# nkkk98/MyGPURaytracer

Hardware: AMD Instinct MI355X
Metric: Mrays/s (higher is better)
Workload: dtype f32; 1 GPU; cornellObj.txt 1920x1080 depth 8, AA on, material sort on, 1 spp/step (BASELINE configs[3] / C4); arith=0, clock_warmup_steps=1152, rccl_ranks=1, parallelism=1 GPU

## Files before the change

### include/mi355x_pathtracer.h

```cpp
#ifndef MI355X_PATHTRACER_H
#define MI355X_PATHTRACER_H

#include <stddef.h>
#include <stdint.h>

#ifdef __cplusplus
extern "C" {
#endif

#define PTX_ABI_VERSION 5
int ptx_abi_version(void);
size_t ptx_sizeof_options(void);
size_t ptx_sizeof_stats(void);

#define PTX_OK 0
#define PTX_ERR_INVALID 1
#define PTX_ERR_IO 2
#define PTX_ERR_HIP 3
#define PTX_ERR_NODEVICE 4
#define PTX_ERR_UNSUPPORTED 5

enum { PTX_SPHERE = 0, PTX_CUBE = 1, PTX_TRIANGLE = 2, PTX_OBJ = 3 };

typedef struct ptx_material {
// ... 212 lines not shown
int  ptx_moments_add(ptx_moments *m, ptx_tracer *t, int64_t samples_total);
int  ptx_moments_add_host(ptx_moments *m, const float *host_rgb_sum, int64_t samples_total);
int  ptx_moments_read(ptx_moments *m, float *mean3, float *cov6, int32_t *batches1, int64_t *samples_out);
int  ptx_moments_summarize(ptx_moments *m, const ptx_moments_params *p, ptx_moments_summary *out);
int  ptx_denoise_measured(ptx_tracer *t, ptx_moments *m, const ptx_denoise_params *dp, const ptx_variance_params *vp, int min_batches,
                          int spp);

int ptx_kat_geom_test(ptx_tracer *t, int geom, int n, const float *rays6, float *out10);
int ptx_kat_obj_tri_test(ptx_tracer *t, int geom, int n, const float *rays6, float *out8);
int ptx_kat_jittered_hemisphere(ptx_tracer *t, int n, const float *normals3, const int32_t *seeds3, int max_iter, float *out3);
int ptx_kat_compute_intersections(ptx_tracer *t, int n, const void *paths44, void *isects32);
int ptx_kat_tile_intersect(ptx_tracer *t, int n, const void *paths44, void *isects32, int split);
int ptx_kat_shade(ptx_tracer *t, int iter, int n, const int32_t *idx, const void *isects32, void *paths44);
int ptx_kat_generate(ptx_tracer *t, int iter, void *paths44);
int ptx_kat_libm(ptx_tracer *t, int n, const float *x, float *sin_out, float *cos_out,
                 const double *pw_in, double *pow5_out, const float *powf_xy, float *powf_out);
int ptx_kat_fast_exact(ptx_tracer *t, int64_t mismatches[3]);
int ptx_debug_tile_geoms(const ptx_camera *camera, int ngeoms, const float *boxes6, int depth_of_field, int tile_rows, int tile_rank,
                         int tile_world, uint32_t *masks_out, int max_tiles);
int ptx_debug_record_masks(int nmaterials, const ptx_material *materials, int ngeoms, const int32_t *geom_type, const int32_t *geom_material,
                           int sort_by_material, uint64_t masks[2]);
int ptx_debug_cull_boxes(int n, const float *boxes6, float *centre_half8);
int ptx_debug_light_bits(int nmaterials, const ptx_material *materials, int ngeoms, const int32_t *geom_material, uint32_t *bits_out);
#define PTX_WALK_LOOP 0
#define PTX_WALK_SKIP 1
#define PTX_WALK_ORDERED 2
#define PTX_WALK_WIDE 3
#define PTX_WALK_WIDE_REFILL 4
int ptx_debug_mesh_plan(ptx_tracer *t, int geom, int32_t out8[8]);
int ptx_debug_bounce_occupancy(ptx_tracer *t, int lds_bytes);
int ptx_debug_aux_nonzero(ptx_tracer *t, int64_t out3[3]);
int ptx_debug_set_capture(ptx_tracer *t, int bounce);
int ptx_debug_bvh_check(const float *faces15, int nfaces, const float *rays6, int nrays, int32_t *face_loop, float *t_loop,
                        int32_t *face_bvh, float *t_bvh, int64_t *stats4);
int ptx_debug_bvh_visits(int64_t out8[8]);
int ptx_debug_read_stamps(ptx_tracer *t, unsigned long long out48[48]);
int ptx_debug_read_stream(ptx_tracer *t, int *n_out, int32_t *pixel_index, int32_t *stream_idx,
                          int32_t *material, float *fields14, int cap);

#ifdef __cplusplus
}
#endif
#endif
```

### mygpuraytracer_amd/api.py

```python
import ctypes as C
import os
import sys
import subprocess

import numpy as np

PKG_DIR = os.path.dirname(os.path.abspath(__file__))
LIB_PATH = os.path.join(PKG_DIR, "libmi355x_pathtracer.so")
if os.environ.get("PTX_AB_LIBRARY"):
    if os.environ.get("PTX_DEV") != "1":
        raise ImportError("PTX_AB_LIBRARY is set (%s) without PTX_DEV=1: variant builds are loaded for A/B timing only; unset it or "
                          "set PTX_DEV=1" % os.environ["PTX_AB_LIBRARY"])
    LIB_PATH = os.path.abspath(os.environ["PTX_AB_LIBRARY"])

PTX_OK = 0
ABI_VERSION = 5
vp = C.c_void_p


class PathTracerError(RuntimeError):
    pass


class Material(C.Structure):
# ... 230 lines not shown
    n = L.ptx_debug_tile_geoms(C.byref(camera), len(b), _ptr(b), int(bool(depth_of_field)), rows, rank, world, _ptr(out), cap)
    if n < 0:
        raise PathTracerError("ptx_debug_tile_geoms: bad argument")
    return out[:n]


def debug_cull_boxes(boxes6):
    L = load_library()
    b = np.ascontiguousarray(boxes6, np.float32).reshape(-1, 6)
    out = np.zeros((len(b), 8), np.float32)
    if L.ptx_debug_cull_boxes(len(b), _ptr(b), _ptr(out)) < 0:
        raise PathTracerError("ptx_debug_cull_boxes: bad argument")
    return out


def debug_light_bits(materials, geom_material):
    L = load_library()
    m = np.ascontiguousarray(materials, np.float32).reshape(-1, 11)
    gm = np.ascontiguousarray(geom_material, np.int32).reshape(-1)
    out = np.zeros(1, np.uint32)
    if L.ptx_debug_light_bits(len(m), _ptr(m), len(gm), _ptr(gm), _ptr(out)) < 0:
        raise PathTracerError("ptx_debug_light_bits: bad argument")
    return int(out[0])


WALK_NAMES = ("loop", "skip", "ordered", "wide", "wide_refill")


def build_library(force=False):
    if force or not os.path.exists(LIB_PATH):
        subprocess.check_call(["make", "-s", "-C", os.path.join(PKG_DIR, "csrc")])
    return LIB_PATH


_lib = None


class Orbit(C.Structure):
    _fields_ = [("phi", C.c_float), ("theta", C.c_float), ("zoom", C.c_float), ("og_look_at", C.c_float * 3)]


def _share_hip_runtime_with_torch():
    import importlib.util
    if "torch" in sys.modules:
        return
    try:
# ... 117 lines not shown
    L.ptx_moments_summarize.restype, L.ptx_moments_summarize.argtypes = i, [vp, C.POINTER(MomentsParams), C.POINTER(MomentsSummary)]
    L.ptx_denoise_measured.restype = i
    L.ptx_denoise_measured.argtypes = [vp, vp, C.POINTER(DenoiseParams), C.POINTER(VarianceParams), i, i]
    L.ptx_get_stats.restype, L.ptx_get_stats.argtypes = i, [vp, C.POINTER(Stats)]
    L.ptx_get_stats_sized.restype, L.ptx_get_stats_sized.argtypes = i, [vp, vp, C.c_size_t]
    L.ptx_owned_pixels.restype, L.ptx_owned_pixels.argtypes = i, [vp]
    L.ptx_stream.restype, L.ptx_stream.argtypes = vp, [vp]
    L.ptx_set_kernel_timing.restype, L.ptx_set_kernel_timing.argtypes = i, [vp, i]
    L.ptx_get_kernel_times.restype, L.ptx_get_kernel_times.argtypes = i, [vp, vp, vp]
    L.ptx_kat_geom_test.restype, L.ptx_kat_geom_test.argtypes = i, [vp, i, i, vp, vp]
    L.ptx_kat_compute_intersections.restype, L.ptx_kat_compute_intersections.argtypes = i, [vp, i, vp, vp]
    L.ptx_kat_obj_tri_test.restype, L.ptx_kat_obj_tri_test.argtypes = i, [vp, i, i, vp, vp]
    L.ptx_kat_jittered_hemisphere.restype, L.ptx_kat_jittered_hemisphere.argtypes = i, [vp, i, vp, vp, i, vp]
    L.ptx_kat_tile_intersect.restype, L.ptx_kat_tile_intersect.argtypes = i, [vp, i, vp, vp, i]
    L.ptx_kat_shade.restype, L.ptx_kat_shade.argtypes = i, [vp, i, i, vp, vp, vp]
    L.ptx_kat_generate.restype, L.ptx_kat_generate.argtypes = i, [vp, i, vp]
    L.ptx_kat_libm.restype, L.ptx_kat_libm.argtypes = i, [vp, i, vp, vp, vp, vp, vp, vp, vp]
    if hasattr(L, "ptx_debug_tile_geoms"):
        L.ptx_debug_tile_geoms.restype, L.ptx_debug_tile_geoms.argtypes = i, [vp, i, vp, i, i, i, i, vp, i]
    if hasattr(L, "ptx_debug_cull_boxes"):
        L.ptx_debug_cull_boxes.restype, L.ptx_debug_cull_boxes.argtypes = i, [i, vp, vp]
    if hasattr(L, "ptx_debug_light_bits"):
        L.ptx_debug_light_bits.restype, L.ptx_debug_light_bits.argtypes = i, [i, vp, i, vp, vp]
    if hasattr(L, "ptx_debug_mesh_plan"):
        L.ptx_debug_mesh_plan.restype, L.ptx_debug_mesh_plan.argtypes = i, [vp, i, vp]
    if hasattr(L, "ptx_kat_fast_exact"):
        L.ptx_kat_fast_exact.restype, L.ptx_kat_fast_exact.argtypes = i, [vp, vp]
    L.ptx_debug_set_capture.restype, L.ptx_debug_set_capture.argtypes = i, [vp, i]
    L.ptx_debug_read_stream.restype, L.ptx_debug_read_stream.argtypes = i, [vp, C.POINTER(i), vp, vp, vp, vp, i]
    L.ptx_multi_create.restype, L.ptx_multi_create.argtypes = i, [vp, C.POINTER(Options), C.POINTER(C.c_int), i, i, C.POINTER(vp)]
    L.ptx_multi_destroy.argtypes = [vp]
    L.ptx_multi_device_count.restype, L.ptx_multi_device_count.argtypes = i, [vp]
    L.ptx_multi_tracer.restype, L.ptx_multi_tracer.argtypes = vp, [vp, i]
    L.ptx_multi_set_camera.restype, L.ptx_multi_set_camera.argtypes = i, [vp, C.POINTER(Camera), i]
    for n in ("ptx_multi_reset_image", "ptx_multi_synchronize", "ptx_multi_assemble"):
        getattr(L, n).restype, getattr(L, n).argtypes = i, [vp]
    L.ptx_multi_iterate.restype, L.ptx_multi_iterate.argtypes = i, [vp, i]
    L.ptx_multi_set_render_ahead.restype, L.ptx_multi_set_render_ahead.argtypes = i, [vp, i]
    L.ptx_multi_render.restype, L.ptx_multi_render.argtypes = i, [vp, i, i]
    L.ptx_multi_device_image.restype, L.ptx_multi_device_image.argtypes = vp, [vp]
    L.ptx_multi_read_image.restype, L.ptx_multi_read_image.argtypes = i, [vp, vp]
    L.ptx_multi_read_albedo.restype, L.ptx_multi_read_albedo.argtypes = i, [vp, vp]
    L.ptx_multi_get_stats.restype, L.ptx_multi_get_stats.argtypes = i, [vp, C.POINTER(Stats)]
    L.ptx_pin_host_buffer.restype, L.ptx_pin_host_buffer.argtypes = i, [vp, C.c_size_t]
    L.ptx_unpin_host_buffer.restype, L.ptx_unpin_host_buffer.argtypes = i, [vp]
    L.sc_cpu_scan.argtypes = [i, vp, vp]
# ... 666 lines not shown
```

### mygpuraytracer_amd/csrc/pt_device.h

```cpp
#pragma once
#include <hip/hip_runtime.h>
#include <stdint.h>

#define PT_DEV __device__ __forceinline__
#define PT_HD __host__ __device__ __forceinline__

#ifndef PT_ARITH
#define PT_ARITH 0
#endif

namespace ptd {

struct vec3 { float x, y, z; };

PT_HD vec3 V3(float x, float y, float z) { vec3 r; r.x = x; r.y = y; r.z = z; return r; }
PT_HD vec3 add(vec3 a, vec3 b) { return V3(a.x + b.x, a.y + b.y, a.z + b.z); }
PT_HD vec3 sub(vec3 a, vec3 b) { return V3(a.x - b.x, a.y - b.y, a.z - b.z); }
PT_HD vec3 mul(vec3 a, vec3 b) { return V3(a.x * b.x, a.y * b.y, a.z * b.z); }
PT_HD vec3 scale(vec3 a, float s) { return V3(a.x * s, a.y * s, a.z * s); }
PT_HD vec3 neg(vec3 a) { return V3(-a.x, -a.y, -a.z); }
PT_HD float dot(vec3 a, vec3 b) { return a.x * b.x + a.y * b.y + a.z * b.z; }
PT_HD vec3 cross(vec3 x, vec3 y) { return V3(x.y * y.z - y.y * x.z, x.z * y.x - y.z * x.x, x.x * y.y - y.x * x.y); }
#ifndef PT_FAST_EXACT
#define PT_FAST_EXACT 1
// ... 249 lines not shown
    const float *__restrict__ tri9;
    const uint8_t *__restrict__ texels;
    int32_t ngeoms, nmats;
    int32_t tri_lds;
    int32_t ntri;
    int32_t ntri_lds;
    const float *__restrict__ gtab;
    const float *__restrict__ aabb;
    uint32_t cube_bits, sphere_bits, mesh_bits;
    uint32_t light_bits;
    const BvhQuad *__restrict__ bvh_nodes;
    const float *__restrict__ bvh_tris;
    const int32_t *__restrict__ bvh_root;
    const int32_t *__restrict__ bvh_depth;
    int32_t bvh_stack;
    const BvhWide4 *__restrict__ bvh_wide;
    const int32_t *__restrict__ bvh_wroot;
    const int32_t *__restrict__ bvh_wneed;
    const float *__restrict__ fnorm;
    const float *__restrict__ cnorm;
    uint32_t bump_bits;
    int32_t mesh_chunks;
    int32_t cull;
    const float *__restrict__ ldsblob;
};

__host__ __device__ constexpr int sceneTableWords(int ntri_lds, int nmats, int ngeoms) { return (ntri_lds * 27 + nmats * 11 + ngeoms * 58 + 3) & ~3; }
PT_DEV int sceneLdsWords(const DScene &sc) { return sceneTableWords(sc.ntri_lds, sc.nmats, sc.ngeoms); }
constexpr int GTAB_WORDS = 40;

extern __shared__ __attribute__((aligned(16))) int32_t pt_lds[];

__device__ __forceinline__ void stageSceneToLds(const DScene &sc, int tid, int nthreads) {
    float *l = reinterpret_cast<float *>(pt_lds);
    if (sc.ldsblob) {
        const int n = sc.ntri_lds * 27 + sc.nmats * 11 + sc.ngeoms * 58;
        for (int k = tid; k < n; k += 4 * nthreads) {
            const int k1 = k + nthreads, k2 = k1 + nthreads, k3 = k2 + nthreads;
            const float a0 = sc.ldsblob[k], a1 = k1 < n ? sc.ldsblob[k1] : 0.f, a2 = k2 < n ? sc.ldsblob[k2] : 0.f, a3 = k3 < n ? sc.ldsblob[k3] : 0.f;
            l[k] = a0;
            if (k1 < n) l[k1] = a1;
            if (k2 < n) l[k2] = a2;
            if (k3 < n) l[k3] = a3;
        }
        return;
    }
    const int n9 = sc.ntri_lds * 9, n15 = sc.ntri_lds * 15, nm = sc.nmats * 11;
// ... 557 lines not shown
    }
    if (hit_geom_index != -1) {
        const DGeom &geom = sc.geoms[hit_geom_index];
        h.t = t_min;
        h.geom = hit_geom_index;
        h.mat = geom.materialid;
        h.u = best.u; h.v = best.v;
        if (geom.type == G_CUBE) h.n = boxNormal(geom, best);
        else if (geom.type == G_SPHERE) h.n = sphereNormal(geom, best);
        else { vec3 geoN; h.n = meshNormal(sc, geom, best, geoN); }
    }
}


PT_HD vec3 mulRows(const float *r, vec3 v, float w) {
    vec3 o;
    o.x = (r[0] * v.x + r[1] * v.y) + (r[2] * v.z + r[3] * w);
    o.y = (r[4] * v.x + r[5] * v.y) + (r[6] * v.z + r[7] * w);
    o.z = (r[8] * v.x + r[9] * v.y) + (r[10] * v.z + r[11] * w);
    return o;
}

constexpr float CULL_FAR_ORIGIN = 1024.0f;
template <bool SUBSET = false>
PT_DEV uint32_t cullMask(const DScene &sc, Ray ray, uint32_t subset = 0xffffffffu) {
    typedef const __attribute__((address_space(4))) float cfloat;
    cfloat *ab = (cfloat *)sc.aabb;
    const float tiny = 1e-20f;
    const float ddx = __builtin_fabsf(ray.d.x) < tiny ? __builtin_copysignf(tiny, ray.d.x) : ray.d.x;
    const float ddy = __builtin_fabsf(ray.d.y) < tiny ? __builtin_copysignf(tiny, ray.d.y) : ray.d.y;
    const float ddz = __builtin_fabsf(ray.d.z) < tiny ? __builtin_copysignf(tiny, ray.d.z) : ray.d.z;
    const float ix = __builtin_amdgcn_rcpf(ddx), iy = __builtin_amdgcn_rcpf(ddy), iz = __builtin_amdgcn_rcpf(ddz);
    const float ox = -(ray.o.x * ix), oy = -(ray.o.y * iy), oz = -(ray.o.z * iz);
    const float ax = __builtin_fabsf(ix), ay = __builtin_fabsf(iy), az = __builtin_fabsf(iz);
    uint32_t mask = 0;
    const int n = sc.ngeoms;
    auto far_origin = [&]() {
        return __builtin_fmaxf(__builtin_fmaxf(__builtin_fabsf(ray.o.x), __builtin_fabsf(ray.o.y)), __builtin_fabsf(ray.o.z)) > CULL_FAR_ORIGIN;
    };
    auto slab = [&](const float *bx) {
        const float mx = __builtin_fmaf(bx[0], ix, ox), my = __builtin_fmaf(bx[1], iy, oy), mz = __builtin_fmaf(bx[2], iz, oz);
        const float x0 = __builtin_fmaf(bx[4], -ax, mx), x1 = __builtin_fmaf(bx[4], ax, mx);
        const float y0 = __builtin_fmaf(bx[5], -ay, my), y1 = __builtin_fmaf(bx[5], ay, my);
        const float z0 = __builtin_fmaf(bx[6], -az, mz), z1 = __builtin_fmaf(bx[6], az, mz);
        const float tn = __builtin_fmaxf(__builtin_fmaxf(x0, y0), z0);
        const float tf = __builtin_fminf(__builtin_fminf(x1, y1), z1);
        return !((tf < tn) || (tf < 0.0f));
    };
    if (SUBSET) {
        uint32_t todo = __builtin_amdgcn_readfirstlane(n >= 32 ? subset : subset & ((1u << n) - 1u));
        while (todo) {
            const int i = __builtin_ctz(todo);
            todo &= todo - 1;
            const int j = todo ? __builtin_ctz(todo) : i;
            todo &= todo - 1;
            float bx[2][8];
#pragma unroll
            for (int k = 0; k < 8; k++) { bx[0][k] = ab[i * 8 + k]; bx[1][k] = ab[j * 8 + k]; }
            mask |= slab(bx[0]) ? (1u << i) : 0u;
            mask |= slab(bx[1]) ? (1u << j) : 0u;
        }
        if (sc.cull > 1 && far_origin()) mask = n >= 32 ? subset : subset & ((1u << n) - 1u);
        return mask;
    }
    int i = n - 1;
    if (n & 1) {
        float bx[8];
#pragma unroll
        for (int k = 0; k < 8; k++) bx[k] = ab[i * 8 + k];
        mask = slab(bx) ? 1u : 0u;
        i--;
    }
    for (; i > 0; i -= 2) {
        float bx[2][8];
#pragma unroll
        for (int k = 0; k < 8; k++) { bx[0][k] = ab[i * 8 + k]; bx[1][k] = ab[(i - 1) * 8 + k]; }
#pragma unroll
        for (int h = 0; h < 2; h++) {
            const unsigned long long verdict = __builtin_amdgcn_ballot_w64(slab(bx[h]));
            asm("v_addc_co_u32_e64 %0, vcc, %0, %0, %1" : "+v"(mask) : "s"(verdict) : "vcc");
        }
    }
    if (sc.cull > 1 && far_origin()) mask = n >= 32 ? 0xffffffffu : (1u << n) - 1u;
    return mask;
}

constexpr unsigned long long KEY_NONE = ~0ull;
PT_DEV unsigned long long packKey(float t, int g, uint32_t aux) {
    return ((unsigned long long)(uint32_t)__float_as_int(t) << 32) | ((unsigned long long)(uint32_t)g << 24) | (aux & 0xffffffu);
}

PT_DEV unsigned long long primKey(const float *gtab, int g, Ray ray) {
    const float *G = gtab + g * GTAB_WORDS;
    float inv[12];
#pragma unroll
    for (int k = 0; k < 12; k++) inv[k] = G[k];
    const int type = __float_as_int(G[36]);
    Ray q;
    q.o = mulRows(inv, ray.o, 1.0f);
    q.d = normalize(mulRows(inv, ray.d, 0.0f));
    vec3 objP = V3(0.f, 0.f, 0.f);
    uint32_t aux = 0;
    bool hit = false;
    if (type == G_CUBE) {
        float tmin = -1e38f, tmax = 1e38f;
// ... 426 lines not shown
```

### mygpuraytracer_amd/csrc/pt_engine.hip

```cpp
#include <hip/hip_runtime.h>
#include <stdint.h>
#include <stdio.h>
#include <string.h>
#include <string>
#include <vector>
#include <algorithm>
#include <cmath>

#include "../../include/mi355x_pathtracer.h"
#include "pt_kernels.h"
#include "pt_scene.h"
#include "pt_denoise.h"

namespace {

thread_local std::string g_last_error;
int set_error(int code, const std::string &msg) { g_last_error = msg; return code; }

#define HIPCHECK(expr)                                                                                   \
    do {                                                                                                 \
        hipError_t e_ = (expr);                                                                          \
        if (e_ != hipSuccess)                                                                            \
            return set_error(PTX_ERR_HIP, std::string(#expr) + ": " + hipGetErrorString(e_));            \
    } while (0)
// ... 205 lines not shown
    hipEvent_t ev_start = nullptr, ev_stop = nullptr;
    bool timing_valid = false;
    ptx_options opt{};
    DCamera cam{};
    int traceDepth = 0;
    TileMap tm{};
    int nbins = 1, nmats = 0, ngeoms = 0, maxTiles = 0, grid = 0, grid_seg = 0, cap = 0, cus = 0;
    bool grid_forced = false;
    int dbg_mesh_wg_per_cu = 0;
    int dbg_extra_lds = 0;
    int dbg_total_wg_per_cu = 0, dbg_nsets = 0;
    DevBuf<DGeom> d_geoms; DevBuf<DMaterial> d_mats; DevBuf<float> d_faces; DevBuf<uint8_t> d_texels;
    float *d_image = nullptr; DevBuf<float> d_image_own;
    DevBuf<float> d_fbuf[3];
    DevBuf<int32_t> d_ibuf[3];
    PathSoA soa[3];
    DevBuf<int32_t> d_counts;
    DevBuf<int32_t> d_chunk;
    DevBuf<int32_t> d_cache_chunk;
    DevBuf<int32_t> d_cache_super;
    int cache_gx = 0;
    DevBuf<int32_t> d_totals;
    int32_t *d_super = nullptr;
    DevBuf<float> d_tri9, d_gtab, d_aabb;
    std::vector<float> h_aabb;
    std::vector<int32_t> h_geom_type, h_roots, h_depths, h_wroots, h_wneeds;
    DevBuf<uint32_t> d_tile_geoms; bool tile_geoms_valid = false;
    DevBuf<BvhQuad> d_bvh_nodes; DevBuf<float> d_bvh_tris; DevBuf<int32_t> d_bvh_root, d_bvh_depth;
    DevBuf<BvhWide4> d_bvh_wide; DevBuf<int32_t> d_bvh_wroot, d_bvh_wneed;
    DevBuf<float> d_fnorm, d_cnorm;
    DevBuf<float> d_ldsblob;
    bool no_fast = false;
    bool no_last = false;
    bool force_fast = false;
    DevBuf<unsigned long long> d_keys; DevBuf<uint32_t> d_items; DevBuf<int32_t> d_item_count;
    DevBuf<int32_t> d_tile_done;
    size_t seg_items = 0;
    int nsuper = 1;
    size_t totals_bytes = 0, seg_totals = 0, field_stride = 0, seg_part = 0;
    int kmax = 1;
    long long split_min_paths = 1LL << 20;
    int lanes = 1;
    hipStream_t lane_stream[MAX_LANES] = {};
    hipEvent_t ev_fork = nullptr, ev_join[MAX_LANES] = {}, ev_chain[MAX_LANES] = {};
    struct Ahead { int first = 0, count = 0, next = 0, unfolded = 0; bool use_cache = false, valid = false, timed = false;
                   unsigned long long dir_bins = ~0ull, ntab_bins = 0ull; };
    Ahead ahead[MAX_LANES];
// ... 15 lines not shown
    DevBuf<float> d_var;
    bool var_done = false;
    DevBuf<unsigned long long> d_stamps;
    DevBuf<float> d_part;
    DevBuf<int32_t> d_cache_totals;
    DevBuf<int32_t> d_emit_count, d_emit_pix; DevBuf<float> d_emit_rgb;
    DevBuf<int64_t> d_stats;
    uint32_t fence_slots = 0;
    int maxBounces = 0;
    bool cache_valid = false;
    int64_t iterations = 0;
    double loop_ms_total = 0.0;
    bool ktiming = false;
    std::vector<hipEvent_t> kev;
    std::vector<int> kev_kind;
    size_t kev_used = 0;
    int capture_bounce = -1;
    DevBuf<int32_t> d_cap;
    DevBuf<float> d_cap_f;
    bool cap_filled = false;
    DScene scene() const {
        DScene s; s.geoms = d_geoms; s.mats = d_mats; s.faces = d_faces; s.tri9 = d_tri9; s.texels = d_texels; s.ngeoms = ngeoms; s.nmats = nmats;
        s.gtab = d_gtab; s.aabb = d_aabb; s.cull = 0; s.cube_bits = cube_bits; s.sphere_bits = sphere_bits; s.mesh_bits = mesh_bits; s.light_bits = light_bits;
        s.bvh_nodes = d_bvh_nodes; s.bvh_tris = d_bvh_tris; s.bvh_root = d_bvh_root; s.bvh_depth = d_bvh_depth; s.bvh_wide = d_bvh_wide; s.bvh_wroot = d_bvh_wroot; s.bvh_wneed = d_bvh_wneed; s.bvh_stack = 0; s.ntri_lds = 0; s.mesh_chunks = mesh_chunks;
        s.fnorm = d_fnorm; s.cnorm = d_cnorm; s.bump_bits = bump_bits;
        s.tri_lds = 0; s.ntri = ntri;
        s.ldsblob = nullptr;
        return s;
    }
    bool cache_active() const { return opt.cache_first_bounce && !opt.antialiasing && !opt.depth_of_field; }
    const KernelSet *ks = static_cast<const KernelSet *>(ptx_arith_kernels_0());
    const LastKernelSet *ksl = static_cast<const LastKernelSet *>(ptx_arith_last_0());
};

namespace {

void carve(PathSoA &s, float *f, int32_t *i, size_t stride) {
    s.q = f; s.i = i; s.stride = (uint32_t)stride;
}

PathSoA soa_shift(PathSoA s, size_t off) {
    s.q += 4 * off; s.i += off;
    return s;
}

void fastdiv_magic(uint32_t d, uint32_t &mul, uint32_t &sh) {
// ... 443 lines not shown
    HC(hipGetDeviceProperties(&prop, dev));
    camera_to_device(*camera, t->cam);
    const int W = t->cam.resx, H = t->cam.resy;
    t->tm.W = W; t->tm.H = H; t->tm.tile_world = opt.tile_world; t->tm.tile_rank = opt.tile_rank;
    t->tm.tile_rows = opt.tile_world > 1 ? opt.tile_rows : H;
    fastdiv_magic((uint32_t)W, t->tm.w_mul, t->tm.w_sh);
    fastdiv_magic((uint32_t)t->tm.tile_rows, t->tm.rows_mul, t->tm.rows_sh);
    t->tm.owned = owned_pixels(W, H, t->tm.tile_rows, opt.tile_rank, opt.tile_world);
    t->maxTiles = (std::max(t->tm.owned, 1) + TILE - 1) / TILE;
    t->cap = t->maxTiles * TILE;
    t->nbins = opt.sort_by_material ? (nmaterials > 0 ? nmaterials : 1) : 1;
    {
        int per_cu = 16;
        if (const char *e = getenv("PTX_DEBUG_WG_PER_CU")) { per_cu = std::max(1, atoi(e)); t->grid_forced = true; }
        t->cus = prop.multiProcessorCount;
        t->grid = std::max(1, std::min(t->maxTiles, prop.multiProcessorCount * per_cu));
    }
    t->grid_seg = std::max(1, std::min(t->grid, t->maxTiles));
    t->nsuper = (t->grid_seg + 63) / 64;
    HostScene hs;
    SceneSwitches sw;
    sw.no_wide_bvh = getenv("PTX_DEBUG_NO_WIDE_BVH") != nullptr; sw.no_chunks = getenv("PTX_DEBUG_NO_CHUNKS") != nullptr;
    sw.no_dir_skip = getenv("PTX_DEBUG_NO_DIR_SKIP") != nullptr; sw.no_normal_codes = getenv("PTX_DEBUG_NO_NORMAL_CODES") != nullptr;
    sw.force_split = getenv("PTX_DEBUG_FORCE_SPLIT") != nullptr;
    if (const int rc = pt_prepare_scene(ngeoms, geoms, nmaterials, materials, opt, t->tm.owned, t->nbins, prop.sharedMemPerBlock, sw, hs)) return fail(rc);
    static_cast<SceneFacts &>(*t) = hs;
    {
        size_t mem_free = 0, mem_total = 0;
        if (opt.batch <= 0 && hipMemGetInfo(&mem_free, &mem_total) != hipSuccess) { mem_free = mem_total = 0; (void)hipGetLastError(); }
        const char *e = getenv("PTX_DEBUG_MEM_BUDGET_MB");
        const LaunchPlan plan = plan_launch_sets(t->tm.owned, t->nbins, t->maxTiles, opt, kmax_cap, mem_free, mem_total, e ? std::max(1LL, atoll(e)) : 0);
        if (!plan.refusal.empty()) { set_error(PTX_ERR_UNSUPPORTED, plan.refusal); return fail(PTX_ERR_UNSUPPORTED); }
        t->kmax = *kmax_used = plan.kmax;
        t->lanes = plan.lanes;
    }
    t->no_fast = getenv("PTX_DEBUG_NO_FAST") != nullptr;
    t->no_last = getenv("PTX_DEBUG_NO_LAST") != nullptr;
    t->force_fast = getenv("PTX_DEBUG_FORCE_FAST") != nullptr;
    if (const char *e = getenv("PTX_DEBUG_TOTAL_WG_PER_CU")) t->dbg_total_wg_per_cu = std::max(0, atoi(e));
    if (const char *e = getenv("PTX_DEBUG_NSETS")) t->dbg_nsets = std::max(0, atoi(e));
    if (const char *e = getenv("PTX_DEBUG_EXTRA_LDS")) t->dbg_extra_lds = std::max(0, std::min(atoi(e), 32768)) & ~15;
    if (const char *e = getenv("PTX_DEBUG_MESH_WG_PER_CU")) t->dbg_mesh_wg_per_cu = std::max(0, atoi(e));
    if (const char *e = getenv("PTX_DEBUG_SPLIT_MIN")) t->split_min_paths = std::max(1LL, atoll(e));
    if (stream) { t->stream = (hipStream_t)stream; t->own_stream = false; }
    else {
        int prio_lo = 0, prio_hi = 0;
        if (hipDeviceGetStreamPriorityRange(&prio_lo, &prio_hi) != hipSuccess) { prio_lo = prio_hi = 0; (void)hipGetLastError(); }
        if (getenv("PTX_DEBUG_NO_PRIORITY")) prio_hi = prio_lo;
        HC(hipStreamCreateWithPriority(&t->stream, hipStreamNonBlocking, prio_hi));
        t->own_stream = true;
    }
    HC(hipEventCreate(&t->ev_start)); HC(hipEventCreate(&t->ev_stop));
    if (t->lanes > 1) {
        HC(hipEventCreateWithFlags(&t->ev_fork, hipEventDisableTiming));
        for (int l = 0; l < t->lanes; l++) {
            if (l) {
                int prio_lo = 0, prio = 0;
                if (hipDeviceGetStreamPriorityRange(&prio_lo, &prio) != hipSuccess || getenv("PTX_DEBUG_NO_PRIORITY")) { prio = 0; (void)hipGetLastError(); }
                if (const char *e = getenv("PTX_DEBUG_LANE_PRIO")) {
                    const char *q = e;
                    for (int k = 1; k <= l && q; k++) { prio = atoi(q); q = strchr(q, ','); if (q) q++; }
                }
                HC(hipStreamCreateWithPriority(&t->lane_stream[l], hipStreamNonBlocking, prio));
            }
            HC(hipEventCreateWithFlags(&t->ev_join[l], hipEventDisableTiming));
            HC(hipEventCreateWithFlags(&t->ev_chain[l], hipEventDisableTiming));
            if (l) { HC(hipEventCreate(&t->ev_ahead0[l])); HC(hipEventCreate(&t->ev_ahead1[l])); }
        }
    }
    HC(t->d_geoms.upload(hs.geoms)); HC(t->d_mats.upload(hs.mats)); HC(t->d_faces.upload(hs.faces)); HC(t->d_texels.upload(hs.texels));
    HC(t->d_tri9.upload(hs.tri9)); HC(t->d_gtab.upload(hs.gtab)); HC(t->d_aabb.upload(hs.aabb_ch));
    HC(t->d_fnorm.upload(hs.fnorm)); HC(t->d_cnorm.upload(hs.cnorm));
    if (t->bvh_meshes) {
        HC(t->d_bvh_nodes.upload(hs.bvh.nodes)); HC(t->d_bvh_tris.upload(hs.bvh.tris));
        HC(t->d_bvh_root.upload(hs.roots)); HC(t->d_bvh_depth.upload(hs.depths));
        if (!hs.bvh.wide.empty()) {
            HC(t->d_bvh_wide.upload(hs.bvh.wide)); HC(t->d_bvh_wroot.upload(hs.wroots)); HC(t->d_bvh_wneed.upload(hs.wneeds));
        }
    }
    if (t->tri_lds) {
        HC(t->d_ldsblob.alloc(std::max<size_t>(hs.ldsblob.size(), 4)));
        if (!hs.ldsblob.empty()) HC(hipMemcpy(t->d_ldsblob, hs.ldsblob.data(), sizeof(float) * hs.ldsblob.size(), hipMemcpyHostToDevice));
    }
    t->h_aabb = std::move(hs.aabb);
    for (const DGeom &g : hs.geoms) t->h_geom_type.push_back(g.type);
    t->h_roots = hs.roots; t->h_depths = hs.depths; t->h_wroots = hs.wroots; t->h_wneeds = hs.wneeds;
    t->h_spec = std::move(hs.h_spec);
    const size_t npix = (size_t)W * H, nseg = (size_t)t->kmax * t->lanes, nb = (size_t)t->nbins;
    if (external_image) t->d_image = external_image;
    else { HC(t->d_image_own.alloc(3 * npix)); HC(t->d_image_own.zero()); t->d_image = t->d_image_own; }
    if (opt.apps_variant) { HC(t->d_albedo.alloc(3 * npix)); HC(t->d_albedo.zero()); }
    t->field_stride = nseg * t->cap;
    for (int k = 0; k < (t->cache_active() ? 3 : 2); k++) {
        const size_t stride = k == 2 ? (size_t)t->cap : t->field_stride;
// ... 837 lines not shown
```

### mygpuraytracer_amd/csrc/pt_scene.h

```cpp
#pragma once
#include "../../include/mi355x_pathtracer.h"
#include "pt_device.h"
#include "pt_bvh.h"

namespace ptd {

struct SceneSwitches {
    bool no_wide_bvh = false;
    bool no_chunks = false;
    bool no_dir_skip = false;
    bool no_normal_codes = false;
    bool force_split = false;
};

struct SceneFacts {
    int ntri = 0, bvh_meshes = 0, bvh_nodes = 0, bvh_stack = BVH_STACK;
    int mesh_chunks = 1;
    int uses_uv = 0;
    uint32_t cube_bits = 0, sphere_bits = 0, mesh_bits = 0;
    uint32_t bump_bits = 0;
    uint32_t light_bits = 0;
    int tri_lds = 0, ntri_lds = 0, cull = 0;
    bool split_mesh = false;
    unsigned long long dir_bins = ~0ull;
    unsigned long long ntab_bins = 0ull;
};

struct HostScene : SceneFacts {
    std::vector<DGeom> geoms;
    std::vector<DMaterial> mats;
    std::vector<float> faces, tri9, gtab, fnorm, cnorm;
    std::vector<uint8_t> texels;
    std::vector<float> aabb, aabb_ch;
    std::vector<uint8_t> h_spec;
    BvhBuild bvh;
    std::vector<int32_t> roots, depths, wroots, wneeds;
    std::vector<float> ldsblob;
};

int pt_prepare_scene(int ngeoms, const ptx_geom *geoms, int nmaterials, const ptx_material *materials, const ptx_options &opt, int owned,
                     int nbins, size_t lds_limit, const SceneSwitches &sw, HostScene &out);

std::vector<float> triangle_table(const float *faces15, int nfaces);
void tile_geom_masks(const DCamera &c, int tile_rows, int tile_rank, int tile_world, int owned, int maxTiles, int ngeoms, const float *aabb8,
                     bool dof, std::vector<uint32_t> &masks);
void camera_to_device(const ptx_camera &c, DCamera &d);
int owned_pixels(int W, int H, int tile_rows, int tile_rank, int tile_world);
uint32_t light_geom_bits(int nmaterials, const DMaterial *mats, int ngeoms, const int32_t *geom_material);

}
```

### mygpuraytracer_amd/csrc/pt_scene.hip

```cpp
#include <string>

#include "pt_scene.h"
#include "pt_kernels.h"

extern "C" void ptx_internal_set_error(const char *msg);

static int set_error(int code, const std::string &msg) { ptx_internal_set_error(msg.c_str()); return code; }

namespace ptd {
void camera_to_device(const ptx_camera &c, DCamera &d) {
    d.resx = c.resolution[0]; d.resy = c.resolution[1];
    memcpy(d.position, c.position, 12); memcpy(d.lookAt, c.lookAt, 12); memcpy(d.view, c.view, 12);
    memcpy(d.up, c.up, 12); memcpy(d.right, c.right, 12); memcpy(d.fov, c.fov, 8); memcpy(d.pixelLength, c.pixelLength, 8);
}

void make_world_aabb(const DGeom &d, const std::vector<float> &faces, float out6[6]) {
    double lo[3] = {1e300, 1e300, 1e300}, hi[3] = {-1e300, -1e300, -1e300};
    bool ok = true;
    auto add = [&](double x, double y, double z) {
        for (int r = 0; r < 3; r++) {
            double v = (double)d.xf[0 * 4 + r] * x + (double)d.xf[1 * 4 + r] * y + (double)d.xf[2 * 4 + r] * z + (double)d.xf[3 * 4 + r];
            if (!(v == v) || v > 1e30 || v < -1e30) ok = false;
            lo[r] = std::min(lo[r], v); hi[r] = std::max(hi[r], v);
        }
// ... 148 lines not shown
    for (int y = 0; y < H; y++) if (tile_world <= 1 || (y / tile_rows) % tile_world == tile_rank) rows++;
    return rows * W;
}

std::vector<float> triangle_table(const float *faces15, int nfaces) {
    std::vector<float> tri9((size_t)std::max(nfaces, 1) * 9, 0.f);
    for (int j = 0; j < nfaces; j++) {
        const float *f = faces15 + (size_t)j * 15;
        float *o = &tri9[(size_t)j * 9];
        for (int k = 0; k < 3; k++) { o[k] = f[k]; o[3 + k] = f[5 + k] - f[k]; o[6 + k] = f[10 + k] - f[k]; }
    }
    return tri9;
}

uint32_t light_geom_bits(int nmaterials, const DMaterial *mats, int ngeoms, const int32_t *geom_material) {
    uint32_t bits = 0;
    for (int g = 0; g < ngeoms && g < 32; g++) {
        const int m = geom_material[g];
        if (m >= 0 && m < nmaterials && mats[m].emittance > 0.0f) bits |= 1u << g;
    }
    return bits;
}

int pt_prepare_scene(int ngeoms, const ptx_geom *geoms, int nmaterials, const ptx_material *materials, const ptx_options &opt, int owned,
                     int nbins, size_t lds_limit, const SceneSwitches &sw, HostScene &hs) {
    hs = HostScene();
    const size_t ng1 = (size_t)std::max(ngeoms, 1);
    hs.geoms.resize(ng1);
    for (int i = 0; i < ngeoms; i++) {
        const ptx_geom &g = geoms[i];
        DGeom &d = hs.geoms[i];
        memset(&d, 0, sizeof d);
        memcpy(d.xf, g.transform, 64); memcpy(d.inv, g.inverseTransform, 64); memcpy(d.invT, g.invTranspose, 64);
        d.type = g.type; d.materialid = g.materialid;
        d.faceStart = (int32_t)(hs.faces.size() / 15); d.faceCount = g.faceSize;
        if (g.faceSize) hs.faces.insert(hs.faces.end(), g.faces, g.faces + (size_t)g.faceSize * 15);
        const ptx_texture *tx[4] = {&g.kd, &g.ks, &g.ke, &g.bump};
        for (int k = 0; k < 4; k++) {
            DTex &dt = d.tex[k];
            if (tx[k]->channels > 0 && tx[k]->image && tx[k]->width > 0 && tx[k]->height > 0) {
                if (tx[k]->channels < 3) return set_error(PTX_ERR_UNSUPPORTED, "textures need >= 3 channels");
                dt.w = tx[k]->width; dt.h = tx[k]->height; dt.ch = tx[k]->channels; dt.off = hs.texels.size();
                hs.uses_uv = 1;
                size_t nbytes = (size_t)dt.w * dt.h * dt.ch;
                hs.texels.insert(hs.texels.end(), tx[k]->image, tx[k]->image + nbytes);
            }
// ... 38 lines not shown
        const DGeom &d = hs.geoms[i];
        float *o = &hs.gtab[(size_t)i * GTAB_WORDS];
        const float *mats3[3] = {d.inv, d.xf, d.invT};
        for (int m = 0; m < 3; m++)
            for (int r = 0; r < 3; r++)
                for (int c = 0; c < 4; c++) o[m * 12 + r * 4 + c] = mats3[m][c * 4 + r];
        int32_t ints[4] = {d.type, d.materialid, d.faceStart, d.faceCount};
        memcpy(o + 36, ints, sizeof ints);
        float box[6];
        make_world_aabb(d, hs.faces, box);
        for (int k = 0; k < 3; k++) { hs.aabb[(size_t)i * 8 + k] = box[k]; hs.aabb[(size_t)i * 8 + 4 + k] = box[3 + k]; }
        if (i < 32) {
            if (d.type == G_OBJ) hs.mesh_bits |= 1u << i;
            else if (d.type == G_CUBE) hs.cube_bits |= 1u << i;
            else if (d.type == G_SPHERE) hs.sphere_bits |= 1u << i;
        }
    }
    hs.aabb_ch.assign(hs.aabb.size(), 0.f);
    for (int i = 0; i < ngeoms; i++) world_box_centre_half(&hs.aabb[(size_t)i * 8], &hs.aabb_ch[(size_t)i * 8]);
    hs.cull = (hs.tri_lds && ngeoms >= 1 && ngeoms <= 32 && !opt.no_cull) ? 1 : 0;
    for (int i = 0; i < ngeoms && hs.cull; i++)
        for (int k = 0; k < 3; k++)
            if (!(std::fabs(hs.aabb[(size_t)i * 8 + k]) <= 0.5f * CULL_FAR_ORIGIN && std::fabs(hs.aabb[(size_t)i * 8 + 4 + k]) <= 0.5f * CULL_FAR_ORIGIN)) hs.cull = 2;
    hs.fnorm.assign((size_t)std::max(hs.ntri, 1) * 3, 0.f); hs.cnorm.assign(ng1 * 18, 0.f);
    for (int i = 0; i < ngeoms; i++) {
        const DGeom &d = hs.geoms[i];
        if (d.type == G_OBJ) {
            if (d.tex[3].ch && i < 32) hs.bump_bits |= 1u << i;
            for (int j = 0; j < d.faceCount; j++) {
                const float *tri = &hs.faces[((size_t)d.faceStart + j) * 15];
                const vec3 e1 = sub(ld3(tri + 5), ld3(tri)), e2 = sub(ld3(tri + 10), ld3(tri));
                const vec3 objN = normalize(cross(e1, e2));
                const vec3 n = normalize(multiplyMV(d.invT, objN, 0.f));
                float *o = &hs.fnorm[((size_t)d.faceStart + j) * 3];
                o[0] = n.x; o[1] = n.y; o[2] = n.z;
            }
        } else if (d.type == G_CUBE) {
            const float *invT = &hs.gtab[(size_t)i * GTAB_WORDS + 24];
            for (int side = 0; side < 6; side++) {
                const int axis = side >> 1;
                const float sgn = (side & 1) ? 1.f : -1.f;
                const vec3 e = V3(axis == 0 ? sgn : 0.f, axis == 1 ? sgn : 0.f, axis == 2 ? sgn : 0.f);
                const vec3 n = normalize(mulRows(invT, e, 0.0f));
                float *o = &hs.cnorm[(size_t)i * 18 + side * 3];
                o[0] = n.x; o[1] = n.y; o[2] = n.z;
            }
// ... 101 lines not shown
    { set_error(PTX_ERR_INVALID, "ptx_debug_record_masks: bad argument"); return -1; }
    unsigned long long d = 0, n = 0;
    record_masks(nmaterials, reinterpret_cast<const DMaterial *>(materials), ngeoms, geom_type, geom_material, sort_by_material != 0, d, n);
    masks[0] = d; masks[1] = n;
    return 0;
}

int ptx_debug_light_bits(int nmaterials, const ptx_material *materials, int ngeoms, const int32_t *geom_material, uint32_t *bits_out) {
    if (nmaterials < 0 || (nmaterials && !materials) || ngeoms < 0 || (ngeoms && !geom_material) || !bits_out)
    { set_error(PTX_ERR_INVALID, "ptx_debug_light_bits: bad argument"); return -1; }
    *bits_out = light_geom_bits(nmaterials, reinterpret_cast<const DMaterial *>(materials), ngeoms, geom_material);
    return 0;
}

int ptx_debug_cull_boxes(int n, const float *boxes6, float *centre_half8) {
    if (n < 0 || (n && (!boxes6 || !centre_half8))) { set_error(PTX_ERR_INVALID, "ptx_debug_cull_boxes: bad argument"); return -1; }
    for (int g = 0; g < n; g++) {
        const float lohi[8] = {boxes6[g * 6], boxes6[g * 6 + 1], boxes6[g * 6 + 2], 0.f, boxes6[g * 6 + 3], boxes6[g * 6 + 4], boxes6[g * 6 + 5], 0.f};
        world_box_centre_half(lohi, centre_half8 + (size_t)g * 8);
    }
    return n;
}

int ptx_debug_tile_geoms(const ptx_camera *camera, int ngeoms, const float *boxes6, int depth_of_field, int tile_rows, int tile_rank, int tile_world,
                         uint32_t *masks_out, int max_tiles) {
    if (!camera || !boxes6 || !masks_out || ngeoms < 1 || ngeoms > 32 || camera->resolution[0] < 1 || camera->resolution[1] < 1)
    { set_error(PTX_ERR_INVALID, "ptx_debug_tile_geoms: bad argument"); return -1; }
    DCamera cam;
    camera_to_device(*camera, cam);
    const int world = tile_world < 1 ? 1 : tile_world, rows = world > 1 ? tile_rows : cam.resy;
    if (world > 1 && (tile_rows < 1 || tile_rank < 0 || tile_rank >= world)) return -1;
    const int owned = owned_pixels(cam.resx, cam.resy, rows, tile_rank, world);
    const int ntiles = (std::max(owned, 1) + TILE - 1) / TILE;
    if (ntiles > max_tiles) return -1;
    std::vector<float> a8((size_t)ngeoms * 8, 0.f);
    for (int g = 0; g < ngeoms; g++)
        for (int k = 0; k < 3; k++) { a8[(size_t)g * 8 + k] = boxes6[g * 6 + k]; a8[(size_t)g * 8 + 4 + k] = boxes6[g * 6 + 3 + k]; }
    std::vector<uint32_t> masks;
    tile_geom_masks(cam, rows, tile_rank, world, owned, ntiles, ngeoms, a8.data(), depth_of_field != 0, masks);
    memcpy(masks_out, masks.data(), sizeof(uint32_t) * (size_t)ntiles);
    return ntiles;
}

int ptx_debug_bvh_visits(int64_t out8[8]) {
    if (!out8) return set_error(PTX_ERR_INVALID, "null argument");
    for (int k = 0; k < 8; k++) out8[k] = g_bvh_visits[k];
// ... 5 lines not shown
```

Before: 42730 Mrays/s.

## Cull OBJ meshes with object-space oriented bounding box tests instead of world AABBs

```diff
diff --git a/include/mi355x_pathtracer.h b/include/mi355x_pathtracer.h
--- a/include/mi355x_pathtracer.h
+++ b/include/mi355x_pathtracer.h
@@ -258,6 +258,7 @@
                            int sort_by_material, uint64_t masks[2]);
 int ptx_debug_cull_boxes(int n, const float *boxes6, float *centre_half8);
 int ptx_debug_light_bits(int nmaterials, const ptx_material *materials, int ngeoms, const int32_t *geom_material, uint32_t *bits_out);
+int ptx_debug_cull_objboxes(int ngeoms, const ptx_geom *geoms, int no_bvh, float margin, float *table16, uint32_t *bits_out);
 #define PTX_WALK_LOOP 0
 #define PTX_WALK_SKIP 1
 #define PTX_WALK_ORDERED 2
diff --git a/mygpuraytracer_amd/api.py b/mygpuraytracer_amd/api.py
--- a/mygpuraytracer_amd/api.py
+++ b/mygpuraytracer_amd/api.py
@@ -276,6 +276,25 @@
     if L.ptx_debug_light_bits(len(m), _ptr(m), len(gm), _ptr(gm), _ptr(out)) < 0:
         raise PathTracerError("ptx_debug_light_bits: bad argument")
     return int(out[0])
+
+
+def debug_cull_objboxes(geom_ints, geom_mats, faces, margin=1.0, no_bvh=0):
+    L = load_library()
+    gi = np.ascontiguousarray(geom_ints, np.int32).reshape(-1, 3)
+    gm = np.ascontiguousarray(geom_mats, np.float32).reshape(-1, 48)
+    keep = [np.ascontiguousarray(f, np.float32).reshape(-1, 15) for f in faces]
+    geoms = (Geom * max(len(gi), 1))()
+    for g in range(len(gi)):
+        geoms[g].type, geoms[g].materialid = int(gi[g][0]), int(gi[g][1])
+        for name, k in (("transform", 0), ("inverseTransform", 16), ("invTranspose", 32)):
+            getattr(geoms[g], name)[:] = gm[g][k:k + 16].tolist()
+        geoms[g].faceSize = len(keep[g])
+        geoms[g].faces = keep[g].ctypes.data_as(C.POINTER(C.c_float)) if len(keep[g]) else None
+    out = np.zeros((len(gi), 16), np.float32)
+    bits = np.zeros(1, np.uint32)
+    if L.ptx_debug_cull_objboxes(len(gi), geoms, int(no_bvh), float(margin), _ptr(out), _ptr(bits)) < 0:
+        raise PathTracerError("ptx_debug_cull_objboxes: bad argument")
+    return out, int(bits[0])
 
 
 WALK_NAMES = ("loop", "skip", "ordered", "wide", "wide_refill")
@@ -439,6 +458,8 @@
         L.ptx_debug_cull_boxes.restype, L.ptx_debug_cull_boxes.argtypes = i, [i, vp, vp]
     if hasattr(L, "ptx_debug_light_bits"):
         L.ptx_debug_light_bits.restype, L.ptx_debug_light_bits.argtypes = i, [i, vp, i, vp, vp]
+    if hasattr(L, "ptx_debug_cull_objboxes"):
+        L.ptx_debug_cull_objboxes.restype, L.ptx_debug_cull_objboxes.argtypes = i, [i, C.POINTER(Geom), i, C.c_float, vp, vp]
     if hasattr(L, "ptx_debug_mesh_plan"):
         L.ptx_debug_mesh_plan.restype, L.ptx_debug_mesh_plan.argtypes = i, [vp, i, vp]
     if hasattr(L, "ptx_kat_fast_exact"):
diff --git a/mygpuraytracer_amd/csrc/pt_device.h b/mygpuraytracer_amd/csrc/pt_device.h
--- a/mygpuraytracer_amd/csrc/pt_device.h
+++ b/mygpuraytracer_amd/csrc/pt_device.h
@@ -295,7 +295,9 @@
     uint32_t bump_bits;
     int32_t mesh_chunks;
     int32_t cull;
+    uint32_t objcull_bits;
     const float *__restrict__ ldsblob;
+    const float *__restrict__ objcull;
 };
 
 __host__ __device__ constexpr int sceneTableWords(int ntri_lds, int nmats, int ngeoms) { return (ntri_lds * 27 + nmats * 11 + ngeoms * 58 + 3) & ~3; }
@@ -899,10 +901,36 @@
 }
 
 constexpr float CULL_FAR_ORIGIN = 1024.0f;
+
+constexpr int OBJCULL_WORDS = 16;
+PT_DEV bool objBoxReach(const __attribute__((address_space(4))) float *T, Ray ray) {
+    const float px = ray.o.x - T[3], py = ray.o.y - T[7], pz = ray.o.z - T[11];
+    const float qx = __builtin_fmaf(T[2], pz, __builtin_fmaf(T[1], py, T[0] * px));
+    const float qy = __builtin_fmaf(T[6], pz, __builtin_fmaf(T[5], py, T[4] * px));
+    const float qz = __builtin_fmaf(T[10], pz, __builtin_fmaf(T[9], py, T[8] * px));
+    const float ex = __builtin_fmaf(T[2], ray.d.z, __builtin_fmaf(T[1], ray.d.y, T[0] * ray.d.x));
+    const float ey = __builtin_fmaf(T[6], ray.d.z, __builtin_fmaf(T[5], ray.d.y, T[4] * ray.d.x));
+    const float ez = __builtin_fmaf(T[10], ray.d.z, __builtin_fmaf(T[9], ray.d.y, T[8] * ray.d.x));
+    const float ax = __builtin_fabsf(qx), ay = __builtin_fabsf(qy), az = __builtin_fabsf(qz);
+    const float s = T[15] * ((ax + ay) + az);
+    const float hx = T[12] + s, hy = T[13] + s, hz = T[14] + s;
+    const float fx = __builtin_fabsf(ex), fy = __builtin_fabsf(ey), fz = __builtin_fabsf(ez);
+    const float floor_ = 0x1p-100f;
+    bool out = (ax > hx) & ((__float_as_int(qx) ^ __float_as_int(ex)) >= 0);
+    out |= (ay > hy) & ((__float_as_int(qy) ^ __float_as_int(ey)) >= 0);
+    out |= (az > hz) & ((__float_as_int(qz) ^ __float_as_int(ez)) >= 0);
+    out |= __builtin_fabsf(__builtin_fmaf(qy, ez, -(qz * ey))) > __builtin_fmaf(hy, fz, __builtin_fmaf(hz, fy, floor_));
+    out |= __builtin_fabsf(__builtin_fmaf(qz, ex, -(qx * ez))) > __builtin_fmaf(hz, fx, __builtin_fmaf(hx, fz, floor_));
+    out |= __builtin_fabsf(__builtin_fmaf(qx, ey, -(qy * ex))) > __builtin_fmaf(hx, fy, __builtin_fmaf(hy, fx, floor_));
+    return !out;
+}
+
 template <bool SUBSET = false>
 PT_DEV uint32_t cullMask(const DScene &sc, Ray ray, uint32_t subset = 0xffffffffu) {
     typedef const __attribute__((address_space(4))) float cfloat;
     cfloat *ab = (cfloat *)sc.aabb;
+    cfloat *oc = (cfloat *)sc.objcull;
+    const uint32_t ocb = sc.objcull_bits;
     const float tiny = 1e-20f;
     const float ddx = __builtin_fabsf(ray.d.x) < tiny ? __builtin_copysignf(tiny, ray.d.x) : ray.d.x;
     const float ddy = __builtin_fabsf(ray.d.y) < tiny ? __builtin_copysignf(tiny, ray.d.y) : ray.d.y;
@@ -924,8 +952,13 @@
         const float tf = __builtin_fminf(__builtin_fminf(x1, y1), z1);
         return !((tf < tn) || (tf < 0.0f));
     };
+    uint32_t om = 0;
+    for (uint32_t todo = __builtin_amdgcn_readfirstlane(SUBSET ? ocb & subset : ocb); todo; todo &= todo - 1) {
+        const int g = __builtin_ctz(todo);
+        om |= objBoxReach(oc + g * OBJCULL_WORDS, ray) ? (1u << g) : 0u;
+    }
     if (SUBSET) {
-        uint32_t todo = __builtin_amdgcn_readfirstlane(n >= 32 ? subset : subset & ((1u << n) - 1u));
+        uint32_t todo = __builtin_amdgcn_readfirstlane((n >= 32 ? subset : subset & ((1u << n) - 1u)) & ~ocb);
         while (todo) {
             const int i = __builtin_ctz(todo);
             todo &= todo - 1;
@@ -937,6 +970,7 @@
             mask |= slab(bx[0]) ? (1u << i) : 0u;
             mask |= slab(bx[1]) ? (1u << j) : 0u;
         }
+        mask |= om;
         if (sc.cull > 1 && far_origin()) mask = n >= 32 ? subset : subset & ((1u << n) - 1u);
         return mask;
     }
@@ -945,7 +979,7 @@
         float bx[8];
 #pragma unroll
         for (int k = 0; k < 8; k++) bx[k] = ab[i * 8 + k];
-        mask = slab(bx) ? 1u : 0u;
+        mask = (!((ocb >> i) & 1u) && slab(bx)) ? 1u : 0u;
         i--;
     }
     for (; i > 0; i -= 2) {
@@ -954,10 +988,11 @@
         for (int k = 0; k < 8; k++) { bx[0][k] = ab[i * 8 + k]; bx[1][k] = ab[(i - 1) * 8 + k]; }
 #pragma unroll
         for (int h = 0; h < 2; h++) {
-            const unsigned long long verdict = __builtin_amdgcn_ballot_w64(slab(bx[h]));
+            const unsigned long long verdict = ((ocb >> (i - h)) & 1u) ? 0ull : __builtin_amdgcn_ballot_w64(slab(bx[h]));
             asm("v_addc_co_u32_e64 %0, vcc, %0, %0, %1" : "+v"(mask) : "s"(verdict) : "vcc");
         }
     }
+    mask |= om;
     if (sc.cull > 1 && far_origin()) mask = n >= 32 ? 0xffffffffu : (1u << n) - 1u;
     return mask;
 }
diff --git a/mygpuraytracer_amd/csrc/pt_engine.hip b/mygpuraytracer_amd/csrc/pt_engine.hip
--- a/mygpuraytracer_amd/csrc/pt_engine.hip
+++ b/mygpuraytracer_amd/csrc/pt_engine.hip
@@ -251,7 +251,7 @@
     int cache_gx = 0;
     DevBuf<int32_t> d_totals;
     int32_t *d_super = nullptr;
-    DevBuf<float> d_tri9, d_gtab, d_aabb;
+    DevBuf<float> d_tri9, d_gtab, d_aabb, d_objcull;
     std::vector<float> h_aabb;
     std::vector<int32_t> h_geom_type, h_roots, h_depths, h_wroots, h_wneeds;
     DevBuf<uint32_t> d_tile_geoms; bool tile_geoms_valid = false;
@@ -313,6 +313,7 @@
     DScene scene() const {
         DScene s; s.geoms = d_geoms; s.mats = d_mats; s.faces = d_faces; s.tri9 = d_tri9; s.texels = d_texels; s.ngeoms = ngeoms; s.nmats = nmats;
         s.gtab = d_gtab; s.aabb = d_aabb; s.cull = 0; s.cube_bits = cube_bits; s.sphere_bits = sphere_bits; s.mesh_bits = mesh_bits; s.light_bits = light_bits;
+        s.objcull = d_objcull; s.objcull_bits = objcull_bits;
         s.bvh_nodes = d_bvh_nodes; s.bvh_tris = d_bvh_tris; s.bvh_root = d_bvh_root; s.bvh_depth = d_bvh_depth; s.bvh_wide = d_bvh_wide; s.bvh_wroot = d_bvh_wroot; s.bvh_wneed = d_bvh_wneed; s.bvh_stack = 0; s.ntri_lds = 0; s.mesh_chunks = mesh_chunks;
         s.fnorm = d_fnorm; s.cnorm = d_cnorm; s.bump_bits = bump_bits;
         s.tri_lds = 0; s.ntri = ntri;
@@ -802,7 +803,7 @@
     SceneSwitches sw;
     sw.no_wide_bvh = getenv("PTX_DEBUG_NO_WIDE_BVH") != nullptr; sw.no_chunks = getenv("PTX_DEBUG_NO_CHUNKS") != nullptr;
     sw.no_dir_skip = getenv("PTX_DEBUG_NO_DIR_SKIP") != nullptr; sw.no_normal_codes = getenv("PTX_DEBUG_NO_NORMAL_CODES") != nullptr;
-    sw.force_split = getenv("PTX_DEBUG_FORCE_SPLIT") != nullptr;
+    sw.force_split = getenv("PTX_DEBUG_FORCE_SPLIT") != nullptr; sw.no_objcull = getenv("PTX_DEBUG_NO_OBJCULL") != nullptr;
     if (const int rc = pt_prepare_scene(ngeoms, geoms, nmaterials, materials, opt, t->tm.owned, t->nbins, prop.sharedMemPerBlock, sw, hs)) return fail(rc);
     static_cast<SceneFacts &>(*t) = hs;
     {
@@ -849,7 +850,7 @@
         }
     }
     HC(t->d_geoms.upload(hs.geoms)); HC(t->d_mats.upload(hs.mats)); HC(t->d_faces.upload(hs.faces)); HC(t->d_texels.upload(hs.texels));
-    HC(t->d_tri9.upload(hs.tri9)); HC(t->d_gtab.upload(hs.gtab)); HC(t->d_aabb.upload(hs.aabb_ch));
+    HC(t->d_tri9.upload(hs.tri9)); HC(t->d_gtab.upload(hs.gtab)); HC(t->d_aabb.upload(hs.aabb_ch)); HC(t->d_objcull.upload(hs.objcull));
     HC(t->d_fnorm.upload(hs.fnorm)); HC(t->d_cnorm.upload(hs.cnorm));
     if (t->bvh_meshes) {
         HC(t->d_bvh_nodes.upload(hs.bvh.nodes)); HC(t->d_bvh_tris.upload(hs.bvh.tris));
diff --git a/mygpuraytracer_amd/csrc/pt_scene.h b/mygpuraytracer_amd/csrc/pt_scene.h
--- a/mygpuraytracer_amd/csrc/pt_scene.h
+++ b/mygpuraytracer_amd/csrc/pt_scene.h
@@ -11,6 +11,7 @@
     bool no_dir_skip = false;
     bool no_normal_codes = false;
     bool force_split = false;
+    bool no_objcull = false;
 };
 
 struct SceneFacts {
@@ -20,6 +21,7 @@
     uint32_t cube_bits = 0, sphere_bits = 0, mesh_bits = 0;
     uint32_t bump_bits = 0;
     uint32_t light_bits = 0;
+    uint32_t objcull_bits = 0;
     int tri_lds = 0, ntri_lds = 0, cull = 0;
     bool split_mesh = false;
     unsigned long long dir_bins = ~0ull;
@@ -32,6 +34,7 @@
     std::vector<float> faces, tri9, gtab, fnorm, cnorm;
     std::vector<uint8_t> texels;
     std::vector<float> aabb, aabb_ch;
+    std::vector<float> objcull;
     std::vector<uint8_t> h_spec;
     BvhBuild bvh;
     std::vector<int32_t> roots, depths, wroots, wneeds;
@@ -47,5 +50,6 @@
 void camera_to_device(const ptx_camera &c, DCamera &d);
 int owned_pixels(int W, int H, int tile_rows, int tile_rank, int tile_world);
 uint32_t light_geom_bits(int nmaterials, const DMaterial *mats, int ngeoms, const int32_t *geom_material);
+bool objcull_entry(const float *inverse16, const float *faces15, int nfaces, double margin, float out16[OBJCULL_WORDS]);
 
 }
diff --git a/mygpuraytracer_amd/csrc/pt_scene.hip b/mygpuraytracer_amd/csrc/pt_scene.hip
--- a/mygpuraytracer_amd/csrc/pt_scene.hip
+++ b/mygpuraytracer_amd/csrc/pt_scene.hip
@@ -194,6 +194,55 @@
     return bits;
 }
 
+bool objcull_entry(const float *inverse16, const float *faces15, int nfaces, double margin, float out16[OBJCULL_WORDS]) {
+    for (int k = 0; k < OBJCULL_WORDS; k++) out16[k] = 0.f;
+    if (!inverse16 || !faces15 || nfaces < 1) return false;
+    double M[3][3], tau[3], lo[3] = {1e300, 1e300, 1e300}, hi[3] = {-1e300, -1e300, -1e300};
+    for (int r = 0; r < 3; r++) { for (int c = 0; c < 3; c++) M[r][c] = inverse16[c * 4 + r]; tau[r] = inverse16[12 + r]; }
+    for (int j = 0; j < nfaces; j++)
+        for (int v = 0; v < 3; v++)
+            for (int r = 0; r < 3; r++) {
+                const double x = faces15[(size_t)j * 15 + v * 5 + r];
+                if (!std::isfinite(x)) return false;
+                lo[r] = std::min(lo[r], x); hi[r] = std::max(hi[r], x);
+            }
+    double I[3][3];
+    const double det = M[0][0] * (M[1][1] * M[2][2] - M[1][2] * M[2][1]) - M[0][1] * (M[1][0] * M[2][2] - M[1][2] * M[2][0]) + M[0][2] * (M[1][0] * M[2][1] - M[1][1] * M[2][0]);
+    if (!std::isfinite(det) || det == 0.0) return false;
+    for (int r = 0; r < 3; r++)
+        for (int c = 0; c < 3; c++) {
+            const int r1 = (c + 1) % 3, r2 = (c + 2) % 3, c1 = (r + 1) % 3, c2 = (r + 2) % 3;
+            I[r][c] = (M[r1][c1] * M[r2][c2] - M[r1][c2] * M[r2][c1]) / det;
+        }
+    double KA = 0.0, KB = 0.0, fro = 0.0;
+    for (int r = 0; r < 3; r++) for (int c = 0; c < 3; c++) fro += I[r][c] * I[r][c];
+    fro = std::sqrt(fro);
+    for (int r = 0; r < 3; r++) {
+        double sum = 0.0;
+        for (int c = 0; c < 3; c++) for (int m = 0; m < 3; m++) sum += std::fabs(M[r][m]) * std::fabs(I[m][c]);
+        KA = std::max(KA, sum);
+        KB = std::max(KB, std::sqrt(M[r][0] * M[r][0] + M[r][1] * M[r][1] + M[r][2] * M[r][2]) * fro);
+    }
+    if (!(KA <= 65536.0 && KB <= 65536.0)) return false;
+    const double u = 1.0 / 16777216.0;
+    double c[3], half[3], R = 0.0, rho = 0.0;
+    float cw[3];
+    for (int r = 0; r < 3; r++) { c[r] = 0.5 * (lo[r] + hi[r]); half[r] = std::max(hi[r] - c[r], c[r] - lo[r]); R += half[r] * half[r]; }
+    R = std::sqrt(R);
+    for (int r = 0; r < 3; r++) cw[r] = (float)(I[r][0] * (c[0] - tau[0]) + I[r][1] * (c[1] - tau[1]) + I[r][2] * (c[2] - tau[2]));
+    for (int r = 0; r < 3; r++) rho = std::max(rho, std::fabs((c[r] - tau[r]) - (M[r][0] * cw[0] + M[r][1] * cw[1] + M[r][2] * cw[2])));
+    const double k = margin * u * (2048.0 + 8.0 * KA + 7.0 * KB + 12.0) / (1.0 - 32.0 * u * (KA + KB));
+    for (int r = 0; r < 3; r++) {
+        const double mcw = std::fabs(M[r][0] * cw[0]) + std::fabs(M[r][1] * cw[1]) + std::fabs(M[r][2] * cw[2]);
+        const double H = half[r] + 4.0 * k * R + margin * 4.0 * u * (mcw + std::fabs(tau[r])) + 2.0 * rho;
+        if (!std::isfinite(H) || H > 0x1p60 || (margin > 0.0 && H < 0x1p-60) || !(std::fabs((double)cw[r]) <= 0x1p60)) { for (int q = 0; q < OBJCULL_WORDS; q++) out16[q] = 0.f; return false; }
+        out16[r * 4 + 0] = (float)M[r][0]; out16[r * 4 + 1] = (float)M[r][1]; out16[r * 4 + 2] = (float)M[r][2]; out16[r * 4 + 3] = cw[r];
+        out16[12 + r] = margin > 0.0 ? nextafterf((float)H, INFINITY) : (float)H;
+    }
+    out16[15] = margin > 0.0 ? nextafterf((float)k, INFINITY) : 0.f;
+    return true;
+}
+
 int pt_prepare_scene(int ngeoms, const ptx_geom *geoms, int nmaterials, const ptx_material *materials, const ptx_options &opt, int owned,
                      int nbins, size_t lds_limit, const SceneSwitches &sw, HostScene &hs) {
     hs = HostScene();
@@ -278,6 +327,11 @@
     for (int i = 0; i < ngeoms && hs.cull; i++)
         for (int k = 0; k < 3; k++)
             if (!(std::fabs(hs.aabb[(size_t)i * 8 + k]) <= 0.5f * CULL_FAR_ORIGIN && std::fabs(hs.aabb[(size_t)i * 8 + 4 + k]) <= 0.5f * CULL_FAR_ORIGIN)) hs.cull = 2;
+    hs.objcull.assign(ng1 * OBJCULL_WORDS, 0.f);
+    if (hs.cull && !hs.bvh_meshes && !sw.no_chunks && !sw.no_objcull)
+        for (int i = 0; i < ngeoms; i++)
+            if (hs.geoms[i].type == G_OBJ && objcull_entry(hs.geoms[i].inv, hs.faces.data() + (size_t)hs.geoms[i].faceStart * 15, hs.geoms[i].faceCount, 1.0, &hs.objcull[(size_t)i * OBJCULL_WORDS]))
+                hs.objcull_bits |= 1u << i;
     hs.fnorm.assign((size_t)std::max(hs.ntri, 1) * 3, 0.f); hs.cnorm.assign(ng1 * 18, 0.f);
     for (int i = 0; i < ngeoms; i++) {
         const DGeom &d = hs.geoms[i];
@@ -425,6 +479,23 @@
     return n;
 }
 
+int ptx_debug_cull_objboxes(int ngeoms, const ptx_geom *geoms, int no_bvh, float margin, float *table16, uint32_t *bits_out) {
+    if (ngeoms < 0 || ngeoms > 32 || (ngeoms && (!geoms || !table16)) || !bits_out || !(margin >= 0.f))
+    { set_error(PTX_ERR_INVALID, "ptx_debug_cull_objboxes: bad argument"); return -1; }
+    bool bvh = false;
+    for (int g = 0; g < ngeoms; g++) {
+        if (geoms[g].faceSize < 0 || (geoms[g].faceSize && !geoms[g].faces)) { set_error(PTX_ERR_INVALID, "ptx_debug_cull_objboxes: bad argument"); return -1; }
+        bvh = bvh || (!no_bvh && geoms[g].type == G_OBJ && geoms[g].faceSize >= BVH_MIN_FACES);
+    }
+    *bits_out = 0;
+    for (int g = 0; g < ngeoms; g++) {
+        for (int k = 0; k < OBJCULL_WORDS; k++) table16[(size_t)g * OBJCULL_WORDS + k] = 0.f;
+        if (!bvh && geoms[g].type == G_OBJ && objcull_entry(geoms[g].inverseTransform, geoms[g].faces, geoms[g].faceSize, margin, table16 + (size_t)g * OBJCULL_WORDS))
+            *bits_out |= 1u << g;
+    }
+    return 0;
+}
+
 int ptx_debug_tile_geoms(const ptx_camera *camera, int ngeoms, const float *boxes6, int depth_of_field, int tile_rows, int tile_rank, int tile_world,
                          uint32_t *masks_out, int max_tiles) {
     if (!camera || !boxes6 || !masks_out || ngeoms < 1 || ngeoms > 32 || camera->resolution[0] < 1 || camera->resolution[1] < 1)
```

Result: faster. 43330 Mrays/s (median of 6 runs) (+1.4%).
